# troyvvgroup/quemb

Hardware: AMD Instinct MI355X
Metric: fragment CCSD iters/sec (full BE sweep over synthetic n_occ=20 n_virt=200 fragments); corr-E error vs oracle in parity_max_abs_err_Eh / parity_n220_abs_err_Eh (higher is better)
Workload: dtype f64

## Files before the change

quemb_amd/csrc/ccsd_ovvv_ops.hip:

```cpp
#include <cstdint>
#include "hip_common.h"

namespace qemb {
namespace ovvv_pass {

typedef double d4 __attribute__((ext_vector_type(4)));
typedef double d2 __attribute__((ext_vector_type(2)));

constexpr int OV_BK = 32;
constexpr int OV_LD = OV_BK + 2;
constexpr int OV_T = 512;
constexpr int OV_WAVES = OV_T / 64;
constexpr int OV_MAXU = CCSD_OVVV_MAX_TILES / OV_WAVES;
constexpr int OV_MAXCH = (16 * CCSD_OVVV_MAX_ROWT * (OV_BK / 2) + OV_T - 1) / OV_T;

struct OvvvArgs {
  const double* ovvv; const double* t1; const double* thk;
  double* zb; double* pa;
  int o, v, rt;
  long long nslab;
};

template <int NT, bool VEC2>
__global__ void __launch_bounds__(OV_T) ccsd_ovvv_pass_kernel(const OvvvArgs g) {
  extern __shared__ __attribute__((aligned(16))) double ov_smem[];
  const int o = g.o, v = g.v, RT = g.rt;
  const int tid = threadIdx.x, lane = tid & 63, l15 = lane & 15, l4 = lane >> 4;
  const int wave = __builtin_amdgcn_readfirstlane(tid >> 6);
  const int rows = 16 * (RT + NT);
  const int items = rows * (OV_BK / 2);
  const int nch = (items + OV_T - 1) / OV_T;
  double* const buf0 = ov_smem;
  double* const buf1 = ov_smem + rows * OV_LD;

  const long long G = gridDim.x, bid = blockIdx.x;
  const long long s_beg = bid * g.nslab / G, s_end = (bid + 1) * g.nslab / G;
  const int nchunk = (v + OV_BK - 1) / OV_BK;
  const long long nstep = (s_end - s_beg) * nchunk;

  const int units = RT * NT, per = (units + OV_WAVES - 1) / OV_WAVES;
  const int u_beg = wave * per < units ? wave * per : units - 1;
  const int cnt = (units - wave * per) < 0 ? 0 : ((units - wave * per) < per ? (units - wave * per) : per);
  const int ct_beg = u_beg / RT, rt_beg = u_beg - ct_beg * RT;
  auto next_tile = [&](int& rt, int& ct) { ++rt; if (rt == RT) { rt = 0; ct = ct + 1 < NT ? ct + 1 : ct; } };
  int a_off[OV_MAXU], b_off[OV_MAXU];
  {
    int rt = rt_beg, ct = ct_beg;
#pragma unroll
    for (int j = 0; j < OV_MAXU; ++j) { a_off[j] = (16 * rt) * OV_LD; b_off[j] = (16 * (RT + ct)) * OV_LD; next_tile(rt, ct); }
  }
  d4 acc[OV_MAXU];
#pragma unroll
  for (int j = 0; j < OV_MAXU; ++j) acc[j] = d4{0.0, 0.0, 0.0, 0.0};

  constexpr int PPR = OV_BK / 2;
  const int p2 = (tid % PPR) * 2;
  int row_off[OV_MAXCH], row_kind[OV_MAXCH];
#pragma unroll
  for (int c = 0; c < OV_MAXCH; ++c) {
    int R = (tid + c * OV_T) / PPR;
    R = R < rows ? R : rows - 1;
    if (R < 16 * RT) { const int a = R < v ? R : v - 1; row_off[c] = a * v; row_kind[c] = 0; }
    else {
      int n = R - 16 * RT;
      n = n < 2 * o ? n : 2 * o - 1;
      row_kind[c] = n < o ? 1 : 2;
      row_off[c] = (n < o ? n : n - o) * v;
    }
  }
  double reg[OV_MAXCH][2];
  int fetched_d = 0;
  auto fetch = [&](long long s, int k0) {
    const double* __restrict__ pA = g.ovvv + s * (long long)v * v;
    const double* __restrict__ pT = g.thk + s * (long long)o * v;
    const int d = k0 + p2;
    fetched_d = d;
#pragma unroll
    for (int c = 0; c < OV_MAXCH; ++c) {
      const double* __restrict__ src = (row_kind[c] == 0 ? pA : row_kind[c] == 1 ? g.t1 : pT) + row_off[c];
      if constexpr (VEC2) {
        const int dc = d < v ? d : v - 2;
        const d2 x = *reinterpret_cast<const d2*>(src + dc);
        reg[c][0] = x[0];
        reg[c][1] = x[1];
      } else {
        const int d0 = d < v ? d : v - 1, d1 = d + 1 < v ? d + 1 : v - 1;
        reg[c][0] = src[d0];
        reg[c][1] = src[d1];
      }
    }
  };
  auto stash = [&](double* __restrict__ S) {
    const bool in0 = fetched_d < v, in1 = fetched_d + 1 < v;
#pragma unroll
    for (int c = 0; c < OV_MAXCH; ++c) {
      const int item = tid + c * OV_T;
      if (c < nch && item < items) *reinterpret_cast<d2*>(S + (item / PPR) * OV_LD + p2) = d2{in0 ? reg[c][0] : 0.0, in1 ? reg[c][1] : 0.0};
    }
  };

  if (nstep > 0) {
    fetch(s_beg, 0);
    stash(buf0);
    __syncthreads();
    long long s = s_beg;
    int ch = 0;
    for (long long t = 0; t < nstep; ++t) {
      {
        const bool last = (t + 1 == nstep);
        const bool wrap = (ch + 1 == nchunk);
        const long long sn = last ? s : (wrap ? s + 1 : s);
        const int chn = last ? ch : (wrap ? 0 : ch + 1);
        fetch(sn, chn * OV_BK);
      }
      const double* __restrict__ S = (t & 1) ? buf1 : buf0;
      const int kleft = v - ch * OV_BK;
      const int nks = ((kleft < OV_BK ? kleft : OV_BK) + 3) >> 2;
      const double* __restrict__ frag = S + l15 * OV_LD + l4;
      auto load_frags = [&](double (&bf)[OV_MAXU], double (&af)[OV_MAXU], int ks) {
#pragma unroll
        for (int j = 0; j < OV_MAXU; ++j) { af[j] = frag[a_off[j] + 4 * ks]; bf[j] = frag[b_off[j] + 4 * ks]; }
      };
      auto mfmas = [&](const double (&bf)[OV_MAXU], const double (&af)[OV_MAXU]) {
#pragma unroll
        for (int j = 0; j < OV_MAXU; ++j)
          if (j < cnt) acc[j] = __builtin_amdgcn_mfma_f64_16x16x4f64(af[j], bf[j], acc[j], 0, 0, 0);
      };
      double bf0[OV_MAXU], af0[OV_MAXU], bf1[OV_MAXU], af1[OV_MAXU];
      load_frags(bf0, af0, 0);
      for (int ks = 0; ks < nks; ks += 2) {
        load_frags(bf1, af1, ks + 1 < nks ? ks + 1 : nks - 1);
        mfmas(bf0, af0);
        if (ks + 1 < nks) {
          load_frags(bf0, af0, ks + 2 < nks ? ks + 2 : nks - 1);
          mfmas(bf1, af1);
        }
      }
      if (ch + 1 == nchunk) {
        double* __restrict__ zb = g.zb + s * (long long)v * o;
        int rt = rt_beg, ct = ct_beg;
#pragma unroll
        for (int j = 0; j < OV_MAXU; ++j) {
          if (j < cnt && 16 * ct < o) {
            const int i = 16 * ct + l15;
#pragma unroll
            for (int r = 0; r < 4; ++r) {
              const int a = 16 * rt + l4 + 4 * r;
              if (a < v && i < o) zb[(long long)a * o + i] = acc[j][r];
              acc[j][r] = (i < o) ? 0.0 : acc[j][r];
            }
          }
          next_tile(rt, ct);
        }
        ch = 0; ++s;
      } else {
        ++ch;
      }
      stash((t & 1) ? buf0 : buf1);
      __syncthreads();
    }
  }
  double* __restrict__ pa = g.pa + bid * (long long)o * v;
  int rt = rt_beg, ct = ct_beg;
#pragma unroll
  for (int j = 0; j < OV_MAXU; ++j) {
    if (j < cnt) {
      const int i = 16 * ct + l15 - o;
#pragma unroll
      for (int r = 0; r < 4; ++r) {
        const int a = 16 * rt + l4 + 4 * r;
        if (a < v && i >= 0 && i < o) pa[(long long)i * v + a] = acc[j][r];
      }
    }
    next_tile(rt, ct);
  }
}

size_t ovvv_lds_bytes(int64_t o, int64_t v) {
  const int64_t rt = (v + 15) / 16, nt = (2 * o + 15) / 16;
  return (size_t)(2 * 16 * (rt + nt) * OV_LD) * sizeof(double);
}

template <int NT, bool VEC2>
int launch_ovvv(const OvvvArgs& a, int G, size_t lds, hipStream_t st) {
  auto kern = ccsd_ovvv_pass_kernel<NT, VEC2>;
  static bool attr_set = false;
  if (!attr_set) {
    HIP_TRY(hipFuncSetAttribute((const void*)kern, hipFuncAttributeMaxDynamicSharedMemorySize, (int)(CCSD_OVVV_MAX_ROWT * 2 * 16 * OV_LD * sizeof(double))));
    attr_set = true;
  }
  return launch("dev_ccsd_ovvv_pass", kern, dim3((unsigned)G), dim3(OV_T), lds, st, a);
}

}
using namespace ovvv_pass;

int dev_ccsd_ovvv_slabs(int64_t o, int64_t v) {
  if (!ccsd_ovvv_shape_ok(o, v)) return 0;
  static const int ncu = [] {
    int dev = 0, n = 0;
    if (hipGetDevice(&dev) != hipSuccess || hipDeviceGetAttribute(&n, hipDeviceAttributeMultiprocessorCount, dev) != hipSuccess || n <= 0) { (void)hipGetLastError(); n = 256; }
    return n;
  }();
  return ncu;
}

int dev_ccsd_ovvv_pass(int64_t o, int64_t v, const double* ovvv, const double* t1, const double* Thk, double* ZB, double* PA) {
  hipStream_t st = hip_stream();
  if (!st) { set_error("libqemb_hip: call qemb_init(device) first"); return QEMB_ERR_DEVICE; }
  if (!ccsd_ovvv_shape_ok(o, v)) { set_error("dev_ccsd_ovvv_pass: shape outside the kernel's limits (ccsd_ovvv_shape_ok)"); return QEMB_ERR_ARG; }
  if (!ovvv || !t1 || !Thk || !ZB || !PA) { set_error("dev_ccsd_ovvv_pass: bad arguments"); return QEMB_ERR_ARG; }
  const int G = dev_ccsd_ovvv_slabs(o, v);
  OvvvArgs a{ovvv, t1, Thk, ZB, PA, (int)o, (int)v, (int)((v + 15) / 16), (long long)(o * v)};
  const size_t lds = ovvv_lds_bytes(o, v);
  const int nt = (int)((2 * o + 15) / 16);
  const bool vec2 = (v % 2) == 0 && (((uintptr_t)ovvv | (uintptr_t)t1 | (uintptr_t)Thk) & 15) == 0;
#define QEMB_OVVV_CASE(N)                                                                                  \
  if (nt == N) return vec2 ? launch_ovvv<N, true>(a, G, lds, st) : launch_ovvv<N, false>(a, G, lds, st);
  QEMB_OVVV_CASE(1)
  QEMB_OVVV_CASE(2)
  QEMB_OVVV_CASE(3)
  QEMB_OVVV_CASE(4)
#undef QEMB_OVVV_CASE
  set_error("dev_ccsd_ovvv_pass: no kernel for this n_occ");
  return QEMB_ERR_ARG;
}

}
```

Baseline: 59.26.

## Restructure ovvv GEMM pipeline with single sync and specialized flagship kernel

Reworks the ovvv pass kernel's main loop. The next chunk is now stashed to shared memory early in the k-loop and its global fetch is issued right after, which removes the trailing stash-plus-barrier at the end of each step and leaves one __syncthreads per step. Row pointers are precomputed and advanced by a stride instead of being rebuilt from slab offsets on every fetch. A compile-time per-wave tile count (PER=5) is added for the n_occ=20, v=200 shape, so accumulator arrays shrink and the cnt guard is dropped. Also adds env-gated diagnostic variants that skip loads or MFMAs, and the reworked overlap depends on correct barrier placement.

```diff
diff --git a/quemb_amd/csrc/ccsd_ovvv_ops.hip b/quemb_amd/csrc/ccsd_ovvv_ops.hip
--- a/quemb_amd/csrc/ccsd_ovvv_ops.hip
+++ b/quemb_amd/csrc/ccsd_ovvv_ops.hip
@@ -21,9 +21,10 @@
   long long nslab;
 };
 
-template <int NT, bool VEC2>
+template <int NT, bool VEC2, int DIAG, int PER>
 __global__ void __launch_bounds__(OV_T) ccsd_ovvv_pass_kernel(const OvvvArgs g) {
   extern __shared__ __attribute__((aligned(16))) double ov_smem[];
+  constexpr int NU = PER ? PER : OV_MAXU;
   const int o = g.o, v = g.v, RT = g.rt;
   const int tid = threadIdx.x, lane = tid & 63, l15 = lane & 15, l4 = lane >> 4;
   const int wave = __builtin_amdgcn_readfirstlane(tid >> 6);
@@ -43,54 +44,55 @@
   const int cnt = (units - wave * per) < 0 ? 0 : ((units - wave * per) < per ? (units - wave * per) : per);
   const int ct_beg = u_beg / RT, rt_beg = u_beg - ct_beg * RT;
   auto next_tile = [&](int& rt, int& ct) { ++rt; if (rt == RT) { rt = 0; ct = ct + 1 < NT ? ct + 1 : ct; } };
-  int a_off[OV_MAXU], b_off[OV_MAXU];
+  int a_off[NU], b_off[NU];
   {
     int rt = rt_beg, ct = ct_beg;
 #pragma unroll
-    for (int j = 0; j < OV_MAXU; ++j) { a_off[j] = (16 * rt) * OV_LD; b_off[j] = (16 * (RT + ct)) * OV_LD; next_tile(rt, ct); }
-  }
-  d4 acc[OV_MAXU];
-#pragma unroll
-  for (int j = 0; j < OV_MAXU; ++j) acc[j] = d4{0.0, 0.0, 0.0, 0.0};
+    for (int j = 0; j < NU; ++j) { a_off[j] = (16 * rt) * OV_LD; b_off[j] = (16 * (RT + ct)) * OV_LD; next_tile(rt, ct); }
+  }
+  d4 acc[NU];
+#pragma unroll
+  for (int j = 0; j < NU; ++j) acc[j] = d4{0.0, 0.0, 0.0, 0.0};
 
   constexpr int PPR = OV_BK / 2;
   const int p2 = (tid % PPR) * 2;
-  int row_off[OV_MAXCH], row_kind[OV_MAXCH];
+  const double* row_ptr[OV_MAXCH];
+  unsigned in_ovvv = 0, in_thk = 0;
 #pragma unroll
   for (int c = 0; c < OV_MAXCH; ++c) {
     int R = (tid + c * OV_T) / PPR;
     R = R < rows ? R : rows - 1;
-    if (R < 16 * RT) { const int a = R < v ? R : v - 1; row_off[c] = a * v; row_kind[c] = 0; }
+    if (R < 16 * RT) { const int a = R < v ? R : v - 1; row_ptr[c] = g.ovvv + (s_beg * v + a) * (long long)v; in_ovvv |= 1u << c; }
     else {
       int n = R - 16 * RT;
       n = n < 2 * o ? n : 2 * o - 1;
-      row_kind[c] = n < o ? 1 : 2;
-      row_off[c] = (n < o ? n : n - o) * v;
+      if (n < o) row_ptr[c] = g.t1 + n * v;
+      else { row_ptr[c] = g.thk + (s_beg * o + (n - o)) * (long long)v; in_thk |= 1u << c; }
     }
   }
   double reg[OV_MAXCH][2];
   int fetched_d = 0;
-  auto fetch = [&](long long s, int k0) {
-    const double* __restrict__ pA = g.ovvv + s * (long long)v * v;
-    const double* __restrict__ pT = g.thk + s * (long long)o * v;
+  auto fetch = [&](int k0) {
     const int d = k0 + p2;
     fetched_d = d;
+    const int dc = d < v ? d : v - 2;
+    const int d0 = d < v ? d : v - 1, d1 = d + 1 < v ? d + 1 : v - 1;
 #pragma unroll
     for (int c = 0; c < OV_MAXCH; ++c) {
-      const double* __restrict__ src = (row_kind[c] == 0 ? pA : row_kind[c] == 1 ? g.t1 : pT) + row_off[c];
-      if constexpr (VEC2) {
-        const int dc = d < v ? d : v - 2;
-        const d2 x = *reinterpret_cast<const d2*>(src + dc);
+      if constexpr (DIAG == 1) {
+        reg[c][0] = 0.0;
+        reg[c][1] = 0.0;
+      } else if constexpr (VEC2) {
+        const d2 x = *reinterpret_cast<const d2*>(row_ptr[c] + dc);
         reg[c][0] = x[0];
         reg[c][1] = x[1];
       } else {
-        const int d0 = d < v ? d : v - 1, d1 = d + 1 < v ? d + 1 : v - 1;
-        reg[c][0] = src[d0];
-        reg[c][1] = src[d1];
+        reg[c][0] = row_ptr[c][d0];
+        reg[c][1] = row_ptr[c][d1];
       }
     }
   };
-  auto stash = [&](double* __restrict__ S) {
+  auto stash = [&](double* S) {
     const bool in0 = fetched_d < v, in1 = fetched_d + 1 < v;
 #pragma unroll
     for (int c = 0; c < OV_MAXCH; ++c) {
@@ -99,48 +101,61 @@
     }
   };
 
-  if (nstep > 0) {
-    fetch(s_beg, 0);
+  struct Frags { double a[NU], b[NU]; };
+  auto run = [&]() {
+    auto load_frags = [&](Frags& f, const double* S) {
+      const double* frag = S + l15 * OV_LD + l4;
+#pragma unroll
+      for (int j = 0; j < NU; ++j) { f.a[j] = frag[a_off[j]]; f.b[j] = frag[b_off[j]]; }
+    };
+    auto mfmas = [&](const Frags& f) {
+#pragma unroll
+      for (int j = 0; j < NU; ++j)
+        if (PER || j < cnt) {
+          if constexpr (DIAG == 2) asm volatile("" ::"v"(f.a[j]), "v"(f.b[j]));
+          else acc[j] = __builtin_amdgcn_mfma_f64_16x16x4f64(f.a[j], f.b[j], acc[j], 0, 0, 0);
+        }
+    };
+    long long tf = 0;
+    int chf = 0;
+    auto fetch_next = [&]() {
+      if (tf + 1 < nstep) {
+        ++tf;
+        if (++chf == nchunk) {
+          chf = 0;
+#pragma unroll
+          for (int c = 0; c < OV_MAXCH; ++c) row_ptr[c] += ((in_ovvv >> c) & 1) ? v * v : ((in_thk >> c) & 1) ? o * v : 0;
+        }
+      }
+      fetch(chf * OV_BK);
+    };
+    fetch(0);
     stash(buf0);
+    fetch_next();
     __syncthreads();
+    Frags f0, f1;
+    load_frags(f0, buf0);
     long long s = s_beg;
     int ch = 0;
     for (long long t = 0; t < nstep; ++t) {
-      {
-        const bool last = (t + 1 == nstep);
-        const bool wrap = (ch + 1 == nchunk);
-        const long long sn = last ? s : (wrap ? s + 1 : s);
-        const int chn = last ? ch : (wrap ? 0 : ch + 1);
-        fetch(sn, chn * OV_BK);
-      }
-      const double* __restrict__ S = (t & 1) ? buf1 : buf0;
+      const double* S = (t & 1) ? buf1 : buf0;
+      double* So = (t & 1) ? buf0 : buf1;
       const int kleft = v - ch * OV_BK;
       const int nks = ((kleft < OV_BK ? kleft : OV_BK) + 3) >> 2;
-      const double* __restrict__ frag = S + l15 * OV_LD + l4;
-      auto load_frags = [&](double (&bf)[OV_MAXU], double (&af)[OV_MAXU], int ks) {
-#pragma unroll
-        for (int j = 0; j < OV_MAXU; ++j) { af[j] = frag[a_off[j] + 4 * ks]; bf[j] = frag[b_off[j] + 4 * ks]; }
-      };
-      auto mfmas = [&](const double (&bf)[OV_MAXU], const double (&af)[OV_MAXU]) {
-#pragma unroll
-        for (int j = 0; j < OV_MAXU; ++j)
-          if (j < cnt) acc[j] = __builtin_amdgcn_mfma_f64_16x16x4f64(af[j], bf[j], acc[j], 0, 0, 0);
-      };
-      double bf0[OV_MAXU], af0[OV_MAXU], bf1[OV_MAXU], af1[OV_MAXU];
-      load_frags(bf0, af0, 0);
-      for (int ks = 0; ks < nks; ks += 2) {
-        load_frags(bf1, af1, ks + 1 < nks ? ks + 1 : nks - 1);
-        mfmas(bf0, af0);
-        if (ks + 1 < nks) {
-          load_frags(bf0, af0, ks + 2 < nks ? ks + 2 : nks - 1);
-          mfmas(bf1, af1);
-        }
+      if (nks == 1) { stash(So); __builtin_amdgcn_sched_barrier(0); fetch_next(); }
+      for (int ks = 0; ks < nks; ++ks) {
+        const bool last = ks + 1 == nks;
+        if (last) __syncthreads();
+        load_frags(f1, last ? So : S + 4 * (ks + 1));
+        mfmas(f0);
+        if (ks == 0 && nks > 1) { stash(So); __builtin_amdgcn_sched_barrier(0); fetch_next(); }
+        f0 = f1;
       }
       if (ch + 1 == nchunk) {
         double* __restrict__ zb = g.zb + s * (long long)v * o;
         int rt = rt_beg, ct = ct_beg;
 #pragma unroll
-        for (int j = 0; j < OV_MAXU; ++j) {
+        for (int j = 0; j < NU; ++j) {
           if (j < cnt && 16 * ct < o) {
             const int i = 16 * ct + l15;
 #pragma unroll
@@ -156,14 +171,15 @@
       } else {
         ++ch;
       }
-      stash((t & 1) ? buf0 : buf1);
-      __syncthreads();
-    }
+    }
+  };
+  if (nstep > 0) {
+    run();
   }
   double* __restrict__ pa = g.pa + bid * (long long)o * v;
   int rt = rt_beg, ct = ct_beg;
 #pragma unroll
-  for (int j = 0; j < OV_MAXU; ++j) {
+  for (int j = 0; j < NU; ++j) {
     if (j < cnt) {
       const int i = 16 * ct + l15 - o;
 #pragma unroll
@@ -181,9 +197,9 @@
   return (size_t)(2 * 16 * (rt + nt) * OV_LD) * sizeof(double);
 }
 
-template <int NT, bool VEC2>
+template <int NT, bool VEC2, int DIAG = 0, int PER = 0>
 int launch_ovvv(const OvvvArgs& a, int G, size_t lds, hipStream_t st) {
-  auto kern = ccsd_ovvv_pass_kernel<NT, VEC2>;
+  auto kern = ccsd_ovvv_pass_kernel<NT, VEC2, DIAG, PER>;
   static bool attr_set = false;
   if (!attr_set) {
     HIP_TRY(hipFuncSetAttribute((const void*)kern, hipFuncAttributeMaxDynamicSharedMemorySize, (int)(CCSD_OVVV_MAX_ROWT * 2 * 16 * OV_LD * sizeof(double))));
@@ -215,6 +231,11 @@
   const size_t lds = ovvv_lds_bytes(o, v);
   const int nt = (int)((2 * o + 15) / 16);
   const bool vec2 = (v % 2) == 0 && (((uintptr_t)ovvv | (uintptr_t)t1 | (uintptr_t)Thk) & 15) == 0;
+  static const int diag = (int)env_int("QEMB_OVVV_DIAGNOSTICS", 0);
+  const bool flagship = nt == 3 && vec2 && a.rt == 13;
+  if (diag == 1 && flagship) return launch_ovvv<3, true, 1, 5>(a, G, lds, st);
+  if (diag == 2 && flagship) return launch_ovvv<3, true, 2, 5>(a, G, lds, st);
+  if (flagship) return launch_ovvv<3, true, 0, 5>(a, G, lds, st);
 #define QEMB_OVVV_CASE(N)                                                                                  \
   if (nt == N) return vec2 ? launch_ovvv<N, true>(a, G, lds, st) : launch_ovvv<N, false>(a, G, lds, st);
   QEMB_OVVV_CASE(1)
```

After: 59.44, median of 6. About the same (+0.3%).
